# lotus-data/lotus

Hardware: NVIDIA H100
Metric: sem_sim_join queries/sec (1M x 768, K=32) (higher is better)
Workload: dtype bf16

## Files before the change

### lotus_b200/csrc/knn_filter_sm90.cu

```cuda
#include <cuda.h>

#include "common.cuh"

namespace b2 {

namespace {

constexpr int BLOCK_M = 128;
constexpr int BLOCK_N = 256;
constexpr int WG_M = 64;
constexpr int KB_BYTES = 64;
constexpr int KSTEPS = 2;
constexpr int STAGE_A_BYTES = BLOCK_M * KB_BYTES;
constexpr int STAGE_B_BYTES = BLOCK_N * KB_BYTES;
constexpr int STAGE_BYTES = STAGE_A_BYTES + STAGE_B_BYTES;
constexpr int NUM_THREADS = 384;
constexpr int CONSUMER_WARPS = 8;
constexpr int MAX_STAGES = 8;
constexpr int SMEM_LIMIT = 232448;
constexpr int SMEM_ALIGN_SLACK = 1024;
constexpr int BAR_BYTES = 256;
constexpr int FILTER_CL = 4;
constexpr int FILTER_CL_MIN_NTILES = 32;
constexpr int FILTER_MAX_K = 1000;

constexpr int PEND = 16;
constexpr int PEND_FLUSH = 8;
__host__ __device__ constexpr int list_set_stride(int kph) { return kph * BLOCK_M + 16; }
constexpr int PEND_SET_STRIDE = PEND * BLOCK_M + 16;
__host__ __device__ constexpr int list_bytes(int kp) { return 2  * 2  * 4 * (list_set_stride(kp / 2) + PEND_SET_STRIDE); }
constexpr int XP_STRIDE = 17;
constexpr int XP_WARP_FLOATS = 16 * XP_STRIDE;
__host__ __device__ constexpr int misc_bytes() { return CONSUMER_WARPS * XP_WARP_FLOATS * 4 + BAR_BYTES + SMEM_ALIGN_SLACK; }
__host__ __device__ constexpr int num_stages(int kp) {
    const int s = (SMEM_LIMIT - list_bytes(kp) - misc_bytes()) / STAGE_BYTES;
    return s > MAX_STAGES ? MAX_STAGES : s;
}
__host__ __device__ constexpr int smem_bytes(int kp) { return num_stages(kp) * STAGE_BYTES + list_bytes(kp) + misc_bytes(); }

__device__ __forceinline__ uint32_t smem_u32(const void* p) { return (uint32_t)__cvta_generic_to_shared(p); }

__device__ __forceinline__ void mbar_init(uint64_t* bar, uint32_t count) {
    asm volatile("mbarrier.init.shared::cta.b64 [%0], %1;" ::"r"(smem_u32(bar)), "r"(count) : "memory");
}
__device__ __forceinline__ void mbar_arrive_expect_tx(uint64_t* bar, uint32_t bytes) {
    asm volatile("mbarrier.arrive.expect_tx.shared::cta.b64 _, [%0], %1;" ::"r"(smem_u32(bar)), "r"(bytes) : "memory");
}
__device__ __forceinline__ void mbar_arrive(uint64_t* bar) {
    asm volatile("mbarrier.arrive.shared::cta.b64 _, [%0];" ::"r"(smem_u32(bar)) : "memory");
}
__device__ __forceinline__ void mbar_arrive_cluster(uint64_t* bar, uint32_t cta) {
    uint32_t remote;
    asm volatile("mapa.shared::cluster.u32 %0, %1, %2;" : "=r"(remote) : "r"(smem_u32(bar)), "r"(cta));
    asm volatile("mbarrier.arrive.shared::cluster.b64 _, [%0];" ::"r"(remote) : "memory");
}
template <bool SUSPEND>
__device__ __forceinline__ void mbar_wait_impl(uint64_t* bar, uint32_t parity) {
    const uint32_t addr = smem_u32(bar);
    uint32_t done = 0;
    uint32_t spins = 0;
    long long t_start = 0;
    while (true) {
        if constexpr (SUSPEND) {
            asm volatile(
                "{\n\t.reg .pred p;\n\t"
                "mbarrier.try_wait.parity.shared::cta.b64 p, [%1], %2, %3;\n\t"
                "selp.u32 %0, 1, 0, p;\n\t}"
                : "=r"(done)
                : "r"(addr), "r"(parity), "r"(20000u)
                : "memory");
        } else {
            asm volatile(
                "{\n\t.reg .pred p;\n\t"
                "mbarrier.try_wait.parity.shared::cta.b64 p, [%1], %2;\n\t"
                "selp.u32 %0, 1, 0, p;\n\t}"
                : "=r"(done)
                : "r"(addr), "r"(parity)
                : "memory");
        }
        if (done) break;
        if ((++spins & 0x3ffu) == 0) {
            const long long now = clock64();
            if (t_start == 0) t_start = now;
            else if (now - t_start > 8000000000LL) __trap();
        }
    }
}
__device__ __forceinline__ void mbar_wait(uint64_t* bar, uint32_t parity) { mbar_wait_impl<true>(bar, parity); }
__device__ __forceinline__ void mbar_wait_spin(uint64_t* bar, uint32_t parity) { mbar_wait_impl<false>(bar, parity); }
__device__ __forceinline__ void fence_barrier_init() { asm volatile("fence.mbarrier_init.release.cluster;" ::: "memory"); }

__device__ __forceinline__ void tma_load_2d(void* smem_dst, const CUtensorMap* tmap, uint64_t* bar, int c0, int c1) {
    asm volatile(
        "cp.async.bulk.tensor.2d.shared::cluster.global.mbarrier::complete_tx::bytes [%0], [%1, {%3, %4}], [%2];" ::"r"(
            smem_u32(smem_dst)),
        "l"(reinterpret_cast<uint64_t>(tmap)), "r"(smem_u32(bar)), "r"(c0), "r"(c1)
        : "memory");
}
__device__ __forceinline__ void tma_load_2d_multicast(void* smem_dst, const CUtensorMap* tmap, uint64_t* bar, int c0, int c1,
                                                      uint16_t mask) {
    asm volatile(
        "cp.async.bulk.tensor.2d.shared::cluster.global.mbarrier::complete_tx::bytes.multicast::cluster [%0], [%1, {%3, %4}], [%2], %5;" ::"r"(
            smem_u32(smem_dst)),
        "l"(reinterpret_cast<uint64_t>(tmap)), "r"(smem_u32(bar)), "r"(c0), "r"(c1), "h"(mask)
        : "memory");
}
__device__ __forceinline__ void tma_prefetch_desc(const CUtensorMap* tmap) {
    asm volatile("prefetch.tensormap [%0];" ::"l"(reinterpret_cast<uint64_t>(tmap)) : "memory");
}
__device__ __forceinline__ uint32_t cluster_ctarank() {
    uint32_t r;
    asm volatile("mov.u32 %0, %%cluster_ctarank;" : "=r"(r));
    return r;
}
__device__ __forceinline__ void cluster_sync_all() {
    asm volatile("barrier.cluster.arrive.release.aligned;\n\tbarrier.cluster.wait.acquire.aligned;" ::: "memory");
}
template <uint32_t N>
__device__ __forceinline__ void setmaxnreg_inc() { asm volatile("setmaxnreg.inc.sync.aligned.u32 %0;" ::"n"(N)); }
template <uint32_t N>
__device__ __forceinline__ void setmaxnreg_dec() { asm volatile("setmaxnreg.dec.sync.aligned.u32 %0;" ::"n"(N)); }

__device__ __forceinline__ uint64_t make_sw64_desc(uint32_t smem_addr) {
    uint64_t desc = 0;
    desc |= (uint64_t)((smem_addr & 0x3FFFFu) >> 4);
    desc |= (uint64_t)1 << 16;
    desc |= (uint64_t)((8 * KB_BYTES) >> 4) << 32;
    desc |= (uint64_t)2 << 62;
    return desc;
}
__device__ __forceinline__ void wgmma_fence() { asm volatile("wgmma.fence.sync.aligned;" ::: "memory"); }
__device__ __forceinline__ void wgmma_commit() { asm volatile("wgmma.commit_group.sync.aligned;" ::: "memory"); }
template <int N>
__device__ __forceinline__ void wgmma_wait() { asm volatile("wgmma.wait_group.sync.aligned %0;" ::"n"(N) : "memory"); }
__device__ __forceinline__ void acc_fence(float (&d)[128]) {
#pragma unroll
    for (int i = 0; i < 128; ++i) asm volatile("" : "+f"(d[i])::"memory");
}

enum class Op { BF16, F16, TF32 };
__host__ __device__ constexpr int op_bytes(Op op) { return op == Op::TF32 ? 4 : 2; }

#define B2_WGMMA_64X256(SHAPE_TYPES, IMM_TAIL)                                                                               \
    asm volatile("{\n\t.reg .pred p;\n\tsetp.ne.b32 p, %130, 0;\n\t"                                                   \
                 "wgmma.mma_async.sync.aligned." SHAPE_TYPES " "                                                           \
                 "{%0, %1, %2, %3, %4, %5, %6, %7, %8, %9, %10, %11, %12, %13, %14, %15, %16, %17, %18, %19, %20, %21, %22, %23, %24, %25, %26, %27, %28, %29, %30, %31, %32, %33, %34, %35, %36, %37, %38, %39, %40, %41, %42, %43, %44, %45, %46, %47, %48, %49, %50, %51, %52, %53, %54, %55, %56, %57, %58, %59, %60, %61, %62, %63, %64, %65, %66, %67, %68, %69, %70, %71, %72, %73, %74, %75, %76, %77, %78, %79, %80, %81, %82, %83, %84, %85, %86, %87, %88, %89, %90, %91, %92, %93, %94, %95, %96, %97, %98, %99, %100, %101, %102, %103, %104, %105, %106, %107, %108, %109, %110, %111, %112, %113, %114, %115, %116, %117, %118, %119, %120, %121, %122, %123, %124, %125, %126, %127}" ", %128, %129, p, 1, 1" IMM_TAIL ";\n\t}"                                                          \
                 : "+f"(d[0]), "+f"(d[1]), "+f"(d[2]), "+f"(d[3]), "+f"(d[4]), "+f"(d[5]), "+f"(d[6]), "+f"(d[7]), "+f"(d[8]), "+f"(d[9]), "+f"(d[10]), "+f"(d[11]), "+f"(d[12]), "+f"(d[13]), "+f"(d[14]), "+f"(d[15]), "+f"(d[16]), "+f"(d[17]), "+f"(d[18]), "+f"(d[19]), "+f"(d[20]), "+f"(d[21]), "+f"(d[22]), "+f"(d[23]), "+f"(d[24]), "+f"(d[25]), "+f"(d[26]), "+f"(d[27]), "+f"(d[28]), "+f"(d[29]), "+f"(d[30]), "+f"(d[31]), "+f"(d[32]), "+f"(d[33]), "+f"(d[34]), "+f"(d[35]), "+f"(d[36]), "+f"(d[37]), "+f"(d[38]), "+f"(d[39]), "+f"(d[40]), "+f"(d[41]), "+f"(d[42]), "+f"(d[43]), "+f"(d[44]), "+f"(d[45]), "+f"(d[46]), "+f"(d[47]), "+f"(d[48]), "+f"(d[49]), "+f"(d[50]), "+f"(d[51]), "+f"(d[52]), "+f"(d[53]), "+f"(d[54]), "+f"(d[55]), "+f"(d[56]), "+f"(d[57]), "+f"(d[58]), "+f"(d[59]), "+f"(d[60]), "+f"(d[61]), "+f"(d[62]), "+f"(d[63]), "+f"(d[64]), "+f"(d[65]), "+f"(d[66]), "+f"(d[67]), "+f"(d[68]), "+f"(d[69]), "+f"(d[70]), "+f"(d[71]), "+f"(d[72]), "+f"(d[73]), "+f"(d[74]), "+f"(d[75]), "+f"(d[76]), "+f"(d[77]), "+f"(d[78]), "+f"(d[79]), "+f"(d[80]), "+f"(d[81]), "+f"(d[82]), "+f"(d[83]), "+f"(d[84]), "+f"(d[85]), "+f"(d[86]), "+f"(d[87]), "+f"(d[88]), "+f"(d[89]), "+f"(d[90]), "+f"(d[91]), "+f"(d[92]), "+f"(d[93]), "+f"(d[94]), "+f"(d[95]), "+f"(d[96]), "+f"(d[97]), "+f"(d[98]), "+f"(d[99]), "+f"(d[100]), "+f"(d[101]), "+f"(d[102]), "+f"(d[103]), "+f"(d[104]), "+f"(d[105]), "+f"(d[106]), "+f"(d[107]), "+f"(d[108]), "+f"(d[109]), "+f"(d[110]), "+f"(d[111]), "+f"(d[112]), "+f"(d[113]), "+f"(d[114]), "+f"(d[115]), "+f"(d[116]), "+f"(d[117]), "+f"(d[118]), "+f"(d[119]), "+f"(d[120]), "+f"(d[121]), "+f"(d[122]), "+f"(d[123]), "+f"(d[124]), "+f"(d[125]), "+f"(d[126]), "+f"(d[127])                                                                                                         \
                 : "l"(adesc), "l"(bdesc), "r"(scale_d))

template <Op OP>
__device__ __forceinline__ void wgmma_64x256(float (&d)[128], uint64_t adesc, uint64_t bdesc, uint32_t scale_d) {
    if constexpr (OP == Op::TF32) {
        B2_WGMMA_64X256("m64n256k8.f32.tf32.tf32", "");
    } else if constexpr (OP == Op::F16) {
        B2_WGMMA_64X256("m64n256k16.f32.f16.f16", ", 0, 0");
    } else {
        B2_WGMMA_64X256("m64n256k16.f32.bf16.bf16", ", 0, 0");
    }
}
#undef B2_WGMMA_64X256

struct FilterParams {
    const float* xnorm;
    float* cand_score;
    int32_t* cand_id;
    float* cand_thr;
    int32_t nq;
    int32_t n;
    int32_t num_kb;
    int32_t n_mtiles;
    int32_t n_munits;
    int32_t n_splits;
    int32_t top1;
    int32_t tiles_per_split;
    int32_t units_whole;
    int32_t n_ntiles;
    int32_t pair_mode, part, nparts, pair_group, pair_items;
    int32_t pair_align;
    float pair_thr;
    int32_t* pair_i;
    int32_t* pair_j;
    unsigned long long* pair_count;
    unsigned long long pair_cap;
};

struct Ring {
    uint8_t* stage_base;
    uint64_t *full_bar, *empty_bar;
};

struct Sched {
    int worker, n_workers;
    int rank;
    int cta;
};
template <int CL>
__device__ __forceinline__ Sched make_sched() {
    Sched sc;
    if constexpr (CL > 1) {
        sc.worker = blockIdx.x >> 1;
        sc.n_workers = gridDim.x >> 1;
        sc.cta = (int)cluster_ctarank();
        sc.rank = CL == 2 ? sc.cta : (sc.cta & 1);
    } else {
        sc.worker = blockIdx.x;
        sc.n_workers = gridDim.x;
        sc.rank = 0;
        sc.cta = 0;
    }
    return sc;
}
__device__ __forceinline__ int num_items(const FilterParams& p) {
    if (p.pair_mode) return p.pair_items;
    return p.units_whole + (p.n_munits - p.units_whole) * p.n_splits;
}
template <int CL>
__device__ __forceinline__ void item_range(const FilterParams& p, const Sched& sc, int item, int& m_tile, int& split, int& t0,
                                           int& t1) {
    if (p.pair_mode) {
        const int grp = item / p.pair_group;
        const int first = (grp * p.nparts + p.part) * p.pair_group;
        const int unit = first + (item - grp * p.pair_group);
        m_tile = CL > 1 ? 2 * unit + sc.rank : unit;
        split = 0;
        const int lead_tile = (p.pair_align ? first : unit) * (CL > 1 ? 2 : 1);
        t0 = (lead_tile * BLOCK_M) / BLOCK_N;
        t1 = p.n_ntiles;
    } else {
        int unit;
        if (item < p.units_whole) {
            unit = item;
            split = 0;
            t0 = 0;
            t1 = p.n_ntiles;
        } else {
            const int j = item - p.units_whole, rem = p.n_munits - p.units_whole;
            unit = p.units_whole + j % rem;
            split = j / rem;
            t0 = split * p.tiles_per_split;
            t1 = min(t0 + p.tiles_per_split, p.n_ntiles);
        }
        m_tile = CL > 1 ? 2 * unit + sc.rank : unit;
    }
}

template <Op OP, int NSTAGES, int CL>
__device__ __forceinline__ void producer_loop(const CUtensorMap* tmap_q, const CUtensorMap* tmap_x, const FilterParams& p,
                                              const Ring& r, const Sched& sc) {
    constexpr int KB_ELEMS = KB_BYTES / op_bytes(OP);
    const int n_items = num_items(p);
    int stage = 0;
    uint32_t phase = 0;
    for (int item = sc.worker; item < n_items; item += sc.n_workers) {
        int m_tile, split, t0, t1;
        item_range<CL>(p, sc, item, m_tile, split, t0, t1);
        for (int t = t0; t < t1; ++t) {
            for (int kb = 0; kb < p.num_kb; ++kb) {
                mbar_wait(&r.empty_bar[stage], phase ^ 1);
                uint8_t* sa = r.stage_base + stage * STAGE_BYTES;
                uint8_t* sb = sa + STAGE_A_BYTES;
                mbar_arrive_expect_tx(&r.full_bar[stage], STAGE_BYTES);
                tma_load_2d(sa, tmap_q, &r.full_bar[stage], kb * KB_ELEMS, m_tile * BLOCK_M);
                if constexpr (CL > 1)
                    tma_load_2d_multicast(sb + sc.cta * (STAGE_B_BYTES / CL), tmap_x, &r.full_bar[stage], kb * KB_ELEMS,
                                          t * BLOCK_N + sc.cta * (BLOCK_N / CL), (uint16_t)((1u << CL) - 1));
                else
                    tma_load_2d(sb, tmap_x, &r.full_bar[stage], kb * KB_ELEMS, t * BLOCK_N);
                if (++stage == NSTAGES) {
                    stage = 0;
                    phase ^= 1;
                }
            }
        }
    }
}

template <int CL>
__device__ __forceinline__ void release_stage(const Ring& r, int s, int cta) {
    __syncwarp();
    if constexpr (CL <= 2) {
        if ((threadIdx.x & 31) == 0) {
            mbar_arrive(&r.empty_bar[s]);
            if constexpr (CL == 2) mbar_arrive_cluster(&r.empty_bar[s], (uint32_t)(cta ^ 1));
        }
    } else {
        const uint32_t lane = threadIdx.x & 31;
        if (lane < CL) mbar_arrive_cluster(&r.empty_bar[s], lane);
    }
}

template <Op OP, int NSTAGES, int CL>
__device__ __forceinline__ void mma_tile(float (&acc)[128], const Ring& r, int num_kb, int g, int cta, int& stage, uint32_t& phase) {
    const uint32_t a_off = (uint32_t)(g * WG_M * KB_BYTES);
    int prev = -1;
    for (int kb = 0; kb < num_kb; ++kb) {
        mbar_wait_spin(&r.full_bar[stage], phase);
        const uint32_t sa = smem_u32(r.stage_base + stage * STAGE_BYTES);
        const uint64_t adesc = make_sw64_desc(sa + a_off);
        const uint64_t bdesc = make_sw64_desc(sa + STAGE_A_BYTES);
        wgmma_fence();
#pragma unroll
        for (int k = 0; k < KSTEPS; ++k)
            wgmma_64x256<OP>(acc, adesc + (uint64_t)(2 * k), bdesc + (uint64_t)(2 * k), (kb | k) != 0 ? 1u : 0u);
        wgmma_commit();
        if (prev >= 0) {
            wgmma_wait<1>();
            release_stage<CL>(r, prev, cta);
        }
        prev = stage;
        if (++stage == NSTAGES) {
            stage = 0;
            phase ^= 1;
        }
    }
    wgmma_wait<0>();
    acc_fence(acc);
    release_stage<CL>(r, prev, cta);
}

template <int NSTAGES, int CL>
__device__ __forceinline__ Ring setup_ring(uint8_t* smem, const CUtensorMap* tmap_q, const CUtensorMap* tmap_x) {
    Ring r;
    r.stage_base = smem;
    uint64_t* bars = reinterpret_cast<uint64_t*>(smem + NSTAGES * STAGE_BYTES);
    r.full_bar = bars;
    r.empty_bar = bars + NSTAGES;
    if (threadIdx.x == 0) {
        tma_prefetch_desc(tmap_q);
        tma_prefetch_desc(tmap_x);
        for (int s = 0; s < NSTAGES; ++s) {
            mbar_init(&r.full_bar[s], 1);
            mbar_init(&r.empty_bar[s], CL * CONSUMER_WARPS);
        }
        fence_barrier_init();
    }
    if constexpr (CL > 1) cluster_sync_all();
    else __syncthreads();
    return r;
}

template <int CL>
__device__ __forceinline__ void teardown_ring() {
    __syncwarp();
    if constexpr (CL > 1) cluster_sync_all();
}

__device__ __forceinline__ uint8_t* align_smem(uint8_t* raw) {
    const uint32_t a = smem_u32(raw);
    return raw + ((1024u - (a & 1023u)) & 1023u);
}

template <int KP>
__device__ __forceinline__ void list_insert(float* sc, int32_t* id, float s, int32_t idx, float& thr, int& minpos) {
    const bool filling = minpos < 0;
    const int pos = filling ? -minpos - 1 : minpos;
    sc[pos * BLOCK_M] = s;
    id[pos * BLOCK_M] = idx;
    if (filling && pos + 1 < KP) {
        minpos = -(pos + 1) - 1;
        return;
    }
    static_assert(KP % 4 == 0, "list length must be a multiple of 4");
    float m[4];
    int mp[4];
#pragma unroll
    for (int c = 0; c < 4; ++c) {
        m[c] = sc[c * BLOCK_M];
        mp[c] = c;
    }
#pragma unroll
    for (int p = 4; p < KP; p += 4) {
#pragma unroll
        for (int c = 0; c < 4; ++c) {
            const float v = sc[(p + c) * BLOCK_M];
            if (v < m[c]) {
                m[c] = v;
                mp[c] = p + c;
            }
        }
    }
    if (m[1] < m[0] || (m[1] == m[0] && mp[1] < mp[0])) { m[0] = m[1]; mp[0] = mp[1]; }
    if (m[3] < m[2] || (m[3] == m[2] && mp[3] < mp[2])) { m[2] = m[3]; mp[2] = mp[3]; }
    if (m[2] < m[0] || (m[2] == m[0] && mp[2] < mp[0])) { m[0] = m[2]; mp[0] = mp[2]; }
    thr = m[0];
    minpos = mp[0];
}

template <int KP>
__device__ __forceinline__ float2 flush_pending(float* my_sc, int32_t* my_id, const float* pend_sc, const int32_t* pend_id,
                                             int cnt, float thr, int minpos) {
    int mx = cnt;
#pragma unroll
    for (int off = 16; off >= 1; off >>= 1) mx = max(mx, __shfl_xor_sync(0xffffffffu, mx, off));
    for (int i = 0; i < mx; ++i) {
        if (i < cnt) {
            const float s = pend_sc[i * BLOCK_M];
            if (s > thr) list_insert<KP>(my_sc, my_id, s, pend_id[i * BLOCK_M], thr, minpos);
        }
        __syncwarp();
    }
    return make_float2(thr, __int_as_float(minpos));
}

template <bool IS_L2>
__device__ __forceinline__ void prepare8(float (&v)[8], int idx0, int valid, const float* xnorm) {
#pragma unroll
    for (int j = 0; j < 8; ++j) {
        if (j < valid) {
            if constexpr (IS_L2) v[j] = fmaf(2.f, v[j], -__ldg(xnorm + idx0 + j));
        } else {
            v[j] = -INFINITY;
        }
    }
}

template <int KPH>
__device__ __forceinline__ void process8(const float (&v)[8], int idx0, float* my_sc, int32_t* my_id, float* pend_sc,
                                         int32_t* pend_id, float& thr, int& minpos, int& cnt) {
#pragma unroll
    for (int j = 0; j < 8; ++j) {
        if (v[j] > thr) {
            pend_sc[cnt * BLOCK_M] = v[j];
            pend_id[cnt * BLOCK_M] = idx0 + j;
            ++cnt;
        }
    }
    if (__any_sync(0xffffffffu, cnt >= PEND_FLUSH)) {
        const float2 fr = flush_pending<KPH>(my_sc, my_id, pend_sc, pend_id, cnt, thr, minpos);
        thr = fr.x;
        minpos = __float_as_int(fr.y);
        cnt = 0;
    }
}

__device__ __forceinline__ void process8_top2(const float (&v)[8], int idx0, float& b1, float& b2, float& b3, int32_t& i1,
                                              int32_t& i2) {
#pragma unroll
    for (int j = 0; j < 8; ++j) {
        const float s = v[j];
        const int32_t id = idx0 + j;
        const bool c3 = s > b3, c2 = s > b2, c1 = s > b1;
        b3 = c2 ? b2 : (c3 ? s : b3);
        i2 = c1 ? i1 : (c2 ? id : i2);
        b2 = c1 ? b1 : (c2 ? s : b2);
        i1 = c1 ? id : i1;
        b1 = c1 ? s : b1;
    }
}

template <int KP, bool IS_L2, Op OP, int CL, bool TOP1 = false>
__global__ void __launch_bounds__(NUM_THREADS, 1)
knn_filter_kernel(const __grid_constant__ CUtensorMap tmap_q, const __grid_constant__ CUtensorMap tmap_x,
                  const FilterParams p) {
    constexpr int NSTAGES = num_stages(KP);
    static_assert(NSTAGES >= 2, "not enough shared memory for the operand ring");
    constexpr int KPH = KP / 2;
    static_assert(KPH % 4 == 0, "list length must allow float4 write-out");
    constexpr int LSET = list_set_stride(KPH);

    extern __shared__ uint8_t smem_raw[];
    uint8_t* smem = align_smem(smem_raw);
    float* xpose = reinterpret_cast<float*>(smem + NSTAGES * STAGE_BYTES + BAR_BYTES);
    float* list_sc = xpose + CONSUMER_WARPS * XP_WARP_FLOATS;
    int32_t* list_id = reinterpret_cast<int32_t*>(list_sc + 2 * LSET);
    float* pend_sc_base = reinterpret_cast<float*>(list_id + 2 * LSET);
    int32_t* pend_id_base = reinterpret_cast<int32_t*>(pend_sc_base + 2 * PEND_SET_STRIDE);
    const int warp = threadIdx.x >> 5;
    const int lane = threadIdx.x & 31;
    const Ring ring = setup_ring<NSTAGES, CL>(smem, &tmap_q, &tmap_x);
    const int n_items = num_items(p);
    const Sched sc = make_sched<CL>();

    if (warp < 4) {
        setmaxnreg_dec<40>();
        if (threadIdx.x == 0) producer_loop<OP, NSTAGES, CL>(&tmap_q, &tmap_x, p, ring, sc);
    } else {
        setmaxnreg_inc<232>();
        const int g = (warp >> 2) - 1;
        const int wq = warp & 3;
        const int rr = lane & 15, e = lane >> 4;
        const int row = g * WG_M + wq * 16 + rr;
        float* my_sc = list_sc + e * LSET + row;
        int32_t* my_id = list_id + e * LSET + row;
        float* pend_sc = pend_sc_base + e * PEND_SET_STRIDE + row;
        int32_t* pend_id = pend_id_base + e * PEND_SET_STRIDE + row;
        float* xs = xpose + (warp - 4) * XP_WARP_FLOATS;
        const int fr = lane >> 2, fc = 2 * (lane & 3);
        int stage = 0;
        uint32_t phase = 0;
        float acc[128];
        for (int item = sc.worker; item < n_items; item += sc.n_workers) {
            int m_tile, split, t0, t1;
            item_range<CL>(p, sc, item, m_tile, split, t0, t1);
            if constexpr (!TOP1) {
#pragma unroll 4
                for (int i = 0; i < KPH; ++i) {
                    my_sc[i * BLOCK_M] = -INFINITY;
                    my_id[i * BLOCK_M] = -1;
                }
            }
            float thr = -INFINITY;
            int minpos = -1;
            int cnt = 0;
            float b1 = -INFINITY, b2 = -INFINITY, b3 = -INFINITY;
            int32_t i1 = -1, i2 = -1;
            float gthr[2][2] = {{-INFINITY, -INFINITY}, {-INFINITY, -INFINITY}};
            for (int t = t0; t < t1; ++t) {
                mma_tile<OP, NSTAGES, CL>(acc, ring, p.num_kb, g, sc.cta, stage, phase);
                const int col0 = t * BLOCK_N;
                const int ncols = min(BLOCK_N, p.n - col0);
#pragma unroll
                for (int c = 0; c < BLOCK_N / 16; ++c) {
                    if constexpr (!TOP1) {
                        bool hit = false;
#pragma unroll
                        for (int jj = 0; jj < 2; ++jj) {
#pragma unroll
                            for (int h = 0; h < 4; ++h) {
                                const int off = 16 * c + 8 * jj + fc + (h & 1);
                                float s = acc[(2 * c + jj) * 4 + h];
                                if constexpr (IS_L2) {
                                    if (off < ncols) s = fmaf(2.f, s, -__ldg(p.xnorm + col0 + off));
                                }
                                hit |= off < ncols && s > gthr[h >> 1][jj];
                            }
                        }
                        if (!__any_sync(0xffffffffu, hit)) continue;
                    }
                    __syncwarp();
#pragma unroll
                    for (int jj = 0; jj < 2; ++jj) {
                        const int a = (2 * c + jj) * 4;
                        xs[fr * XP_STRIDE + 8 * jj + fc] = acc[a];
                        xs[fr * XP_STRIDE + 8 * jj + fc + 1] = acc[a + 1];
                        xs[(fr + 8) * XP_STRIDE + 8 * jj + fc] = acc[a + 2];
                        xs[(fr + 8) * XP_STRIDE + 8 * jj + fc + 1] = acc[a + 3];
                    }
                    __syncwarp();
                    float v[8];
#pragma unroll
                    for (int j = 0; j < 8; ++j) v[j] = xs[rr * XP_STRIDE + 8 * e + j];
                    const int off = 16 * c + 8 * e;
                    prepare8<IS_L2>(v, col0 + off, ncols - off, p.xnorm);
                    if constexpr (TOP1) {
                        process8_top2(v, col0 + off, b1, b2, b3, i1, i2);
                    } else {
                        process8<KPH>(v, col0 + off, my_sc, my_id, pend_sc, pend_id, thr, minpos, cnt);
#pragma unroll
                        for (int h = 0; h < 2; ++h) {
#pragma unroll
                            for (int s = 0; s < 2; ++s) gthr[h][s] = __shfl_sync(0xffffffffu, thr, fr + 8 * h + 16 * s);
                        }
                    }
                }
            }
            if constexpr (TOP1) {
#pragma unroll 4
                for (int i = 2; i < KPH; ++i) {
                    my_sc[i * BLOCK_M] = -INFINITY;
                    my_id[i * BLOCK_M] = -1;
                }
                my_sc[0 * BLOCK_M] = b1;
                my_id[0 * BLOCK_M] = i1;
                my_sc[1 * BLOCK_M] = b2;
                my_id[1 * BLOCK_M] = i2;
                thr = b3;
            } else {
                const float2 fl = flush_pending<KPH>(my_sc, my_id, pend_sc, pend_id, cnt, thr, minpos);
                thr = fl.x;
                minpos = __float_as_int(fl.y);
                cnt = 0;
            }
            const int q = m_tile * BLOCK_M + row;
            if (q < p.nq) {
                const size_t lidx = ((size_t)q * p.n_splits + split) * 2 + e;
                float4* osc = reinterpret_cast<float4*>(p.cand_score + lidx * KPH);
                int4* oid = reinterpret_cast<int4*>(p.cand_id + lidx * KPH);
#pragma unroll 4
                for (int i = 0; i < KPH / 4; ++i) {
                    osc[i] = make_float4(my_sc[(4 * i + 0) * BLOCK_M], my_sc[(4 * i + 1) * BLOCK_M],
                                         my_sc[(4 * i + 2) * BLOCK_M], my_sc[(4 * i + 3) * BLOCK_M]);
                    oid[i] = make_int4(my_id[(4 * i + 0) * BLOCK_M], my_id[(4 * i + 1) * BLOCK_M],
                                       my_id[(4 * i + 2) * BLOCK_M], my_id[(4 * i + 3) * BLOCK_M]);
                }
                p.cand_thr[lidx] = thr;
            }
        }
    }

    teardown_ring<CL>();
}

constexpr int PAIR_STAGES = MAX_STAGES;
constexpr int PAIR_SMEM = PAIR_STAGES * STAGE_BYTES + BAR_BYTES + SMEM_ALIGN_SLACK;

template <Op OP, int CL>
__global__ void __launch_bounds__(NUM_THREADS, 1)
pair_filter_kernel(const __grid_constant__ CUtensorMap tmap_q, const __grid_constant__ CUtensorMap tmap_x, const FilterParams p) {
    extern __shared__ uint8_t smem_raw[];
    uint8_t* smem = align_smem(smem_raw);
    const int warp = threadIdx.x >> 5;
    const int lane = threadIdx.x & 31;
    const Ring ring = setup_ring<PAIR_STAGES, CL>(smem, &tmap_q, &tmap_x);
    const int n_items = num_items(p);
    const Sched sc = make_sched<CL>();
    if (warp < 4) {
        setmaxnreg_dec<40>();
        if (threadIdx.x == 0) producer_loop<OP, PAIR_STAGES, CL>(&tmap_q, &tmap_x, p, ring, sc);
    } else {
        setmaxnreg_inc<232>();
        const int g = (warp >> 2) - 1;
        const int wq = warp & 3;
        const float thr = p.pair_thr;
        int stage = 0;
        uint32_t phase = 0;
        float acc[128];
        for (int item = sc.worker; item < n_items; item += sc.n_workers) {
            int m_tile, split, t0, t1;
            item_range<CL>(p, sc, item, m_tile, split, t0, t1);
            const int gi0 = m_tile * BLOCK_M + g * WG_M + wq * 16 + (lane >> 2);
            for (int t = t0; t < t1; ++t) {
                mma_tile<OP, PAIR_STAGES, CL>(acc, ring, p.num_kb, g, sc.cta, stage, phase);
                const int col0 = t * BLOCK_N + 2 * (lane & 3);
                float mx = acc[0];
#pragma unroll
                for (int i = 1; i < 128; ++i) mx = fmaxf(mx, acc[i]);
                if (mx > thr && gi0 < p.n) {
#pragma unroll
                    for (int i = 0; i < 128; ++i) {
                        const int gi = gi0 + 8 * ((i >> 1) & 1);
                        const int gj = col0 + 8 * (i >> 2) + (i & 1);
                        if (acc[i] > thr && gj > gi && gj < p.n && gi < p.n) {
                            const unsigned long long pos = atomicAdd(p.pair_count, 1ull);
                            if (pos < p.pair_cap) {
                                p.pair_i[pos] = gi;
                                p.pair_j[pos] = gj;
                            }
                        }
                    }
                }
            }
        }
    }
    teardown_ring<CL>();
}

typedef CUresult (*PFN_encodeTiled)(CUtensorMap*, CUtensorMapDataType, cuuint32_t, void*, const cuuint64_t*,
                                    const cuuint64_t*, const cuuint32_t*, const cuuint32_t*, CUtensorMapInterleave,
                                    CUtensorMapSwizzle, CUtensorMapL2promotion, CUtensorMapFloatOOBfill);

PFN_encodeTiled get_encode_fn() {
    static PFN_encodeTiled fn = nullptr;
    if (fn) return fn;
    void* p = nullptr;
    cudaDriverEntryPointQueryResult qres;
    cudaError_t e = cudaGetDriverEntryPoint("cuTensorMapEncodeTiled", &p, cudaEnableDefault, &qres);
    if (e != cudaSuccess || qres != cudaDriverEntryPointSuccess || !p) {
        set_error("cuTensorMapEncodeTiled is not available from the driver (%s)", cudaGetErrorString(e));
        return nullptr;
    }
    fn = reinterpret_cast<PFN_encodeTiled>(p);
    return fn;
}

Op filter_op(int filt_dtype) {
    switch (filt_dtype) {
        case B2_F32: return Op::TF32;
        case B2_BF16: return Op::BF16;
        default: return Op::F16;
    }
}
CUtensorMapDataType tma_data_type(Op op) {
    switch (op) {
        case Op::TF32: return CU_TENSOR_MAP_DATA_TYPE_FLOAT32;
        case Op::BF16: return CU_TENSOR_MAP_DATA_TYPE_BFLOAT16;
        default: return CU_TENSOR_MAP_DATA_TYPE_FLOAT16;
    }
}

int make_tmap(CUtensorMap* map, const void* base, Op op, int64_t rows, int64_t cols, int64_t pitch, int box_rows) {
    PFN_encodeTiled enc = get_encode_fn();
    if (!enc) return B2_ECUDA;
    const int esz = op_bytes(op);
    cuuint64_t gdim[2] = {(cuuint64_t)cols, (cuuint64_t)rows};
    cuuint64_t gstride[1] = {(cuuint64_t)pitch * esz};
    cuuint32_t box[2] = {(cuuint32_t)(KB_BYTES / esz), (cuuint32_t)box_rows};
    cuuint32_t estr[2] = {1, 1};
    if ((reinterpret_cast<uintptr_t>(base) & 15) != 0 || (gstride[0] & 15) != 0) {
        set_error("TMA operand not 16-byte aligned (base %p, pitch %lld B)", base, (long long)gstride[0]);
        return B2_EINVAL;
    }
    CUresult r = enc(map, tma_data_type(op), 2,
                     const_cast<void*>(base), gdim, gstride, box, estr, CU_TENSOR_MAP_INTERLEAVE_NONE,
                     CU_TENSOR_MAP_SWIZZLE_64B, CU_TENSOR_MAP_L2_PROMOTION_L2_256B, CU_TENSOR_MAP_FLOAT_OOB_FILL_NONE);
    if (r != CUDA_SUCCESS) {
        set_error("cuTensorMapEncodeTiled failed with CUresult %d (rows %lld cols %lld pitch %lld)", (int)r,
                  (long long)rows, (long long)cols, (long long)pitch);
        return B2_ECUDA;
    }
    return B2_OK;
}

template <typename Kern>
int launch_cluster(Kern kern, int grid, int smem, int cl, const CUtensorMap& tq, const CUtensorMap& tx, const FilterParams& p,
                   cudaStream_t stream) {
    B2_CUDA(cudaFuncSetAttribute(kern, cudaFuncAttributeMaxDynamicSharedMemorySize, smem));
    cudaLaunchConfig_t cfg = {};
    cfg.gridDim = dim3((unsigned)grid);
    cfg.blockDim = dim3(NUM_THREADS);
    cfg.dynamicSmemBytes = smem;
    cfg.stream = stream;
    cudaLaunchAttribute attr[1];
    attr[0].id = cudaLaunchAttributeClusterDimension;
    attr[0].val.clusterDim.x = (unsigned)cl;
    attr[0].val.clusterDim.y = 1;
    attr[0].val.clusterDim.z = 1;
    cfg.attrs = attr;
    cfg.numAttrs = 1;
    B2_CUDA(cudaLaunchKernelEx(&cfg, kern, tq, tx, p));
    B2_LAUNCH_CHECK();
    g_stats[ST_FILTER_LAUNCHES]++;
    return B2_OK;
}

template <int KP, bool IS_L2, Op OP, int CL, bool TOP1 = false>
int launch_variant(const CUtensorMap& tq, const CUtensorMap& tx, const FilterParams& p, int grid, cudaStream_t stream) {
    return launch_cluster(knn_filter_kernel<KP, IS_L2, OP, CL, TOP1>, grid, smem_bytes(KP), CL, tq, tx, p, stream);
}

template <int KP, bool IS_L2, int CL, bool TOP1 = false>
int launch_op(Op op, const CUtensorMap& tq, const CUtensorMap& tx, const FilterParams& p, int grid, cudaStream_t stream) {
    switch (op) {
        case Op::TF32: return launch_variant<KP, IS_L2, Op::TF32, CL, TOP1>(tq, tx, p, grid, stream);
        case Op::BF16: return launch_variant<KP, IS_L2, Op::BF16, CL, TOP1>(tq, tx, p, grid, stream);
        default: return launch_variant<KP, IS_L2, Op::F16, CL, TOP1>(tq, tx, p, grid, stream);
    }
}

template <int KP, int CL>
int launch_kp(bool is_l2, Op op, const CUtensorMap& tq, const CUtensorMap& tx, const FilterParams& p, int grid,
              cudaStream_t stream) {
    return is_l2 ? launch_op<KP, true, CL>(op, tq, tx, p, grid, stream) : launch_op<KP, false, CL>(op, tq, tx, p, grid, stream);
}

template <int CL>
int launch_top1(bool is_l2, Op op, const CUtensorMap& tq, const CUtensorMap& tx, const FilterParams& p, int grid,
                cudaStream_t stream) {
    return is_l2 ? launch_op<16, true, CL, true>(op, tq, tx, p, grid, stream)
                 : launch_op<16, false, CL, true>(op, tq, tx, p, grid, stream);
}

template <int CL>
int launch_cl(int kp, bool is_l2, Op op, const CUtensorMap& tq, const CUtensorMap& tx, const FilterParams& p, int grid,
              cudaStream_t stream) {
    switch (kp) {
        case 16: return launch_kp<16, CL>(is_l2, op, tq, tx, p, grid, stream);
        case 32: return launch_kp<32, CL>(is_l2, op, tq, tx, p, grid, stream);
        case 64: return launch_kp<64, CL>(is_l2, op, tq, tx, p, grid, stream);
        case 72: return launch_kp<72, CL>(is_l2, op, tq, tx, p, grid, stream);
        default: set_error("internal: unsupported candidate capacity %d", kp); return B2_EINVAL;
    }
}

template <typename Kern>
int co_resident_clusters(Kern kern, int smem, int cl, int* n) {
    B2_CUDA(cudaFuncSetAttribute(kern, cudaFuncAttributeMaxDynamicSharedMemorySize, smem));
    cudaLaunchConfig_t cfg = {};
    cfg.gridDim = dim3((unsigned)cl);
    cfg.blockDim = dim3(NUM_THREADS);
    cfg.dynamicSmemBytes = smem;
    cudaLaunchAttribute attr[1];
    attr[0].id = cudaLaunchAttributeClusterDimension;
    attr[0].val.clusterDim.x = (unsigned)cl;
    attr[0].val.clusterDim.y = 1;
    attr[0].val.clusterDim.z = 1;
    cfg.attrs = attr;
    cfg.numAttrs = 1;
    *n = 0;
    B2_CUDA(cudaOccupancyMaxActiveClusters(n, kern, &cfg));
    if (*n <= 0) {
        set_error("the filter kernel fits no cluster of %d CTAs (%d B of shared memory each)", cl, smem);
        return B2_ECUDA;
    }
    return B2_OK;
}

template <int KP>
int co_resident_filter_clusters(int cl, int* n) {
    switch (cl) {
        case 1: return co_resident_clusters(knn_filter_kernel<KP, false, Op::BF16, 1>, smem_bytes(KP), cl, n);
        case 2: return co_resident_clusters(knn_filter_kernel<KP, false, Op::BF16, 2>, smem_bytes(KP), cl, n);
        default: return co_resident_clusters(knn_filter_kernel<KP, false, Op::BF16, FILTER_CL>, smem_bytes(KP), cl, n);
    }
}

}

int sm_count(int device) {
    static int cached[64] = {0};
    if (device >= 0 && device < 64 && cached[device]) return cached[device];
    int n = 132;
    cudaDeviceGetAttribute(&n, cudaDevAttrMultiProcessorCount, device);
    if (device >= 0 && device < 64) cached[device] = n;
    return n;
}

int filter_kp_for_k(int k) {
    if (k <= 6) return 16;
    if (k <= 16) return 32;
    if (k <= 40) return 64;
    if (k <= FILTER_MAX_K) return 72;
    return 0;
}

int filter_min_splits_for_k(int k) { return k <= 40 ? 1 : (int)ceil_div(k, 36); }

int filter_cluster(int64_t nq, int64_t n, bool top1) {
    static int mode = -1;
    if (mode < 0) {
        const char* e = getenv("B2_FILTER_2CTA");
        mode = e ? (atoi(e) != 0 ? 1 : 0) : 1;
    }
    const int cl = top1 || ceil_div(n, BLOCK_N) < FILTER_CL_MIN_NTILES ? 2 : FILTER_CL;
    return mode == 1 && ceil_div(nq, BLOCK_M) >= cl ? cl : 1;
}

int filter_workers(int device, int kp, int cl, int* workers) {
    static int cached[64][3][4] = {};
    const int ki = kp == 16 ? 0 : kp == 32 ? 1 : kp == 64 ? 2 : 3;
    const int ci = cl == 1 ? 0 : cl == 2 ? 1 : 2;
    int* slot = (device >= 0 && device < 64) ? &cached[device][ci][ki] : nullptr;
    if (slot && *slot) {
        *workers = *slot;
        return B2_OK;
    }
    switch (kp) {
        case 16: B2_TRY(co_resident_filter_clusters<16>(cl, workers)); break;
        case 32: B2_TRY(co_resident_filter_clusters<32>(cl, workers)); break;
        case 64: B2_TRY(co_resident_filter_clusters<64>(cl, workers)); break;
        case 72: B2_TRY(co_resident_filter_clusters<72>(cl, workers)); break;
        default: set_error("internal: unsupported candidate capacity %d", kp); return B2_EINVAL;
    }
    if (cl > 2) *workers *= cl / 2;
    if (slot) *slot = *workers;
    return B2_OK;
}

int filter_choose_splits(int64_t nq, int64_t n, int workers, int cl, bool top1, int min_splits, int* units_whole) {
    if (units_whole) *units_whole = 0;
    const int64_t n_mtiles = ceil_div(nq, BLOCK_M);
    const int64_t n_units = cl > 1 ? ceil_div(n_mtiles, 2) : n_mtiles;
    auto split_units = [cl](int64_t u) { return cl > 2 ? u + (u & 1) : u; };
    const int64_t n_ntiles = ceil_div(n, BLOCK_N);
    const double kWarmupTiles = top1 ? 1.0 : 13.0;
    double best_cost = 1e300;
    int best = 0;
    for (int s = std::max(1, min_splits); s <= 256 && s <= n_ntiles; ++s) {
        const int64_t tps = ceil_div(n_ntiles, s);
        if (ceil_div(n_ntiles, tps) != s) continue;
        const int64_t items = split_units(n_units) * s;
        const int64_t waves = ceil_div(items, workers);
        const double cost = (double)waves * ((double)tps + kWarmupTiles) * (1.0 + 0.004 * s);
        if (cost < best_cost - 1e-9) {
            best_cost = cost;
            best = s;
        }
    }
    const int64_t waves_a = n_units / workers;
    if (units_whole && min_splits <= 1 && waves_a >= 1) {
        const int64_t ua = waves_a * workers, rem = n_units - ua;
        const double cost_a = (double)waves_a * ((double)n_ntiles + kWarmupTiles);
        double best2 = 1e300;
        int s2 = 1;
        if (rem == 0) {
            best2 = cost_a;
        } else {
            for (int s = 1; s <= 256 && s <= n_ntiles; ++s) {
                const int64_t tps = ceil_div(n_ntiles, s);
                if (ceil_div(n_ntiles, tps) != s) continue;
                const int64_t waves_b = ceil_div(split_units(rem) * s, workers);
                const double cost = (cost_a + (double)waves_b * ((double)tps + kWarmupTiles)) * (1.0 + 0.002 * s);
                if (cost < best2 - 1e-9) {
                    best2 = cost;
                    s2 = s;
                }
            }
        }
        if (best2 < best_cost - 1e-9) {
            *units_whole = (int)ua;
            return s2;
        }
    }
    return best;
}

int launch_knn_filter(const MatView& X, const void* q_filt, int64_t q_pitch, int64_t nq, int metric, int kp,
                      int n_splits, int cluster, int workers, float* cand_score, int32_t* cand_id, float* cand_thr,
                      cudaStream_t stream, bool top1, int units_whole) {
    if (nq <= 0 || X.n <= 0) return B2_OK;
    if (X.n > 0x7fffff00LL || nq > 0x7fffff00LL) {
        set_error("matrix too large for 32-bit row ids (n=%lld nq=%lld)", (long long)X.n, (long long)nq);
        return B2_ERANGE;
    }
    const Op op = filter_op(X.filt_dtype);
    const int kb_elems = KB_BYTES / op_bytes(op);
    CUtensorMap tq, tx;
    const int64_t op_cols = X.d;
    B2_TRY(make_tmap(&tq, q_filt, op, nq, op_cols, q_pitch, BLOCK_M));
    B2_TRY(make_tmap(&tx, X.filt, op, X.n, op_cols, X.filt_pitch, BLOCK_N / cluster));
    FilterParams p;
    p.xnorm = X.norm2;
    p.cand_score = cand_score;
    p.cand_id = cand_id;
    p.cand_thr = cand_thr;
    p.nq = (int32_t)nq;
    p.n = (int32_t)X.n;
    p.num_kb = (int32_t)ceil_div(X.d, kb_elems);
    p.n_mtiles = (int32_t)ceil_div(nq, BLOCK_M);
    p.n_munits = cluster > 1 ? (p.n_mtiles + 1) / 2 : p.n_mtiles;
    p.n_ntiles = (int32_t)ceil_div(X.n, BLOCK_N);
    p.tiles_per_split = (int32_t)ceil_div(p.n_ntiles, n_splits);
    p.n_splits = n_splits;
    p.units_whole = units_whole;
    p.top1 = (top1 && kp == 16) ? 1 : 0;
    p.pair_mode = 0;
// ... 110 lines not shown
```

Measured before the change: 266,400.

## Keep query A-fragments register-resident across N tiles via RS wgmma

```diff
diff --git a/lotus_b200/csrc/knn_filter_sm90.cu b/lotus_b200/csrc/knn_filter_sm90.cu
--- a/lotus_b200/csrc/knn_filter_sm90.cu
+++ b/lotus_b200/csrc/knn_filter_sm90.cu
@@ -11,6 +11,7 @@
 constexpr int WG_M = 64;
 constexpr int KB_BYTES = 64;
 constexpr int KSTEPS = 2;
+constexpr int KB_AREGS = 4 * KSTEPS;
 constexpr int STAGE_A_BYTES = BLOCK_M * KB_BYTES;
 constexpr int STAGE_B_BYTES = BLOCK_N * KB_BYTES;
 constexpr int STAGE_BYTES = STAGE_A_BYTES + STAGE_B_BYTES;
@@ -22,6 +23,7 @@
 constexpr int BAR_BYTES = 256;
 constexpr int FILTER_CL = 4;
 constexpr int FILTER_CL_MIN_NTILES = 32;
+constexpr int FILTER_RES_KB = 6;
 constexpr int FILTER_MAX_K = 1000;
 
 constexpr int PEND = 16;
@@ -141,12 +143,21 @@
 enum class Op { BF16, F16, TF32 };
 __host__ __device__ constexpr int op_bytes(Op op) { return op == Op::TF32 ? 4 : 2; }
 
+#define B2_WGMMA_D                                                                                                           \
+    "{%0, %1, %2, %3, %4, %5, %6, %7, %8, %9, %10, %11, %12, %13, %14, %15, %16, %17, %18, %19, %20, %21, %22, %23, %24, %25, %26, %27, %28, %29, %30, %31, %32, %33, %34, %35, %36, %37, %38, %39, %40, %41, %42, %43, %44, %45, %46, %47, %48, %49, %50, %51, %52, %53, %54, %55, %56, %57, %58, %59, %60, %61, %62, %63, %64, %65, %66, %67, %68, %69, %70, %71, %72, %73, %74, %75, %76, %77, %78, %79, %80, %81, %82, %83, %84, %85, %86, %87, %88, %89, %90, %91, %92, %93, %94, %95, %96, %97, %98, %99, %100, %101, %102, %103, %104, %105, %106, %107, %108, %109, %110, %111, %112, %113, %114, %115, %116, %117, %118, %119, %120, %121, %122, %123, %124, %125, %126, %127}"
+#define B2_WGMMA_D_OPS                                                                                                       \
+    "+f"(d[0]), "+f"(d[1]), "+f"(d[2]), "+f"(d[3]), "+f"(d[4]), "+f"(d[5]), "+f"(d[6]), "+f"(d[7]), "+f"(d[8]), "+f"(d[9]), "+f"(d[10]), "+f"(d[11]), "+f"(d[12]), "+f"(d[13]), "+f"(d[14]), "+f"(d[15]), "+f"(d[16]), "+f"(d[17]), "+f"(d[18]), "+f"(d[19]), "+f"(d[20]), "+f"(d[21]), "+f"(d[22]), "+f"(d[23]), "+f"(d[24]), "+f"(d[25]), "+f"(d[26]), "+f"(d[27]), "+f"(d[28]), "+f"(d[29]), "+f"(d[30]), "+f"(d[31]), "+f"(d[32]), "+f"(d[33]), "+f"(d[34]), "+f"(d[35]), "+f"(d[36]), "+f"(d[37]), "+f"(d[38]), "+f"(d[39]), "+f"(d[40]), "+f"(d[41]), "+f"(d[42]), "+f"(d[43]), "+f"(d[44]), "+f"(d[45]), "+f"(d[46]), "+f"(d[47]), "+f"(d[48]), "+f"(d[49]), "+f"(d[50]), "+f"(d[51]), "+f"(d[52]), "+f"(d[53]), "+f"(d[54]), "+f"(d[55]), "+f"(d[56]), "+f"(d[57]), "+f"(d[58]), "+f"(d[59]), "+f"(d[60]), "+f"(d[61]), "+f"(d[62]), "+f"(d[63]), "+f"(d[64]), "+f"(d[65]), "+f"(d[66]), "+f"(d[67]), "+f"(d[68]), "+f"(d[69]), "+f"(d[70]), "+f"(d[71]), "+f"(d[72]), "+f"(d[73]), "+f"(d[74]), "+f"(d[75]), "+f"(d[76]), "+f"(d[77]), "+f"(d[78]), "+f"(d[79]), "+f"(d[80]), "+f"(d[81]), "+f"(d[82]), "+f"(d[83]), "+f"(d[84]), "+f"(d[85]), "+f"(d[86]), "+f"(d[87]), "+f"(d[88]), "+f"(d[89]), "+f"(d[90]), "+f"(d[91]), "+f"(d[92]), "+f"(d[93]), "+f"(d[94]), "+f"(d[95]), "+f"(d[96]), "+f"(d[97]), "+f"(d[98]), "+f"(d[99]), "+f"(d[100]), "+f"(d[101]), "+f"(d[102]), "+f"(d[103]), "+f"(d[104]), "+f"(d[105]), "+f"(d[106]), "+f"(d[107]), "+f"(d[108]), "+f"(d[109]), "+f"(d[110]), "+f"(d[111]), "+f"(d[112]), "+f"(d[113]), "+f"(d[114]), "+f"(d[115]), "+f"(d[116]), "+f"(d[117]), "+f"(d[118]), "+f"(d[119]), "+f"(d[120]), "+f"(d[121]), "+f"(d[122]), "+f"(d[123]), "+f"(d[124]), "+f"(d[125]), "+f"(d[126]), "+f"(d[127])
 #define B2_WGMMA_64X256(SHAPE_TYPES, IMM_TAIL)                                                                               \
     asm volatile("{\n\t.reg .pred p;\n\tsetp.ne.b32 p, %130, 0;\n\t"                                                   \
-                 "wgmma.mma_async.sync.aligned." SHAPE_TYPES " "                                                           \
-                 "{%0, %1, %2, %3, %4, %5, %6, %7, %8, %9, %10, %11, %12, %13, %14, %15, %16, %17, %18, %19, %20, %21, %22, %23, %24, %25, %26, %27, %28, %29, %30, %31, %32, %33, %34, %35, %36, %37, %38, %39, %40, %41, %42, %43, %44, %45, %46, %47, %48, %49, %50, %51, %52, %53, %54, %55, %56, %57, %58, %59, %60, %61, %62, %63, %64, %65, %66, %67, %68, %69, %70, %71, %72, %73, %74, %75, %76, %77, %78, %79, %80, %81, %82, %83, %84, %85, %86, %87, %88, %89, %90, %91, %92, %93, %94, %95, %96, %97, %98, %99, %100, %101, %102, %103, %104, %105, %106, %107, %108, %109, %110, %111, %112, %113, %114, %115, %116, %117, %118, %119, %120, %121, %122, %123, %124, %125, %126, %127}" ", %128, %129, p, 1, 1" IMM_TAIL ";\n\t}"                                                          \
-                 : "+f"(d[0]), "+f"(d[1]), "+f"(d[2]), "+f"(d[3]), "+f"(d[4]), "+f"(d[5]), "+f"(d[6]), "+f"(d[7]), "+f"(d[8]), "+f"(d[9]), "+f"(d[10]), "+f"(d[11]), "+f"(d[12]), "+f"(d[13]), "+f"(d[14]), "+f"(d[15]), "+f"(d[16]), "+f"(d[17]), "+f"(d[18]), "+f"(d[19]), "+f"(d[20]), "+f"(d[21]), "+f"(d[22]), "+f"(d[23]), "+f"(d[24]), "+f"(d[25]), "+f"(d[26]), "+f"(d[27]), "+f"(d[28]), "+f"(d[29]), "+f"(d[30]), "+f"(d[31]), "+f"(d[32]), "+f"(d[33]), "+f"(d[34]), "+f"(d[35]), "+f"(d[36]), "+f"(d[37]), "+f"(d[38]), "+f"(d[39]), "+f"(d[40]), "+f"(d[41]), "+f"(d[42]), "+f"(d[43]), "+f"(d[44]), "+f"(d[45]), "+f"(d[46]), "+f"(d[47]), "+f"(d[48]), "+f"(d[49]), "+f"(d[50]), "+f"(d[51]), "+f"(d[52]), "+f"(d[53]), "+f"(d[54]), "+f"(d[55]), "+f"(d[56]), "+f"(d[57]), "+f"(d[58]), "+f"(d[59]), "+f"(d[60]), "+f"(d[61]), "+f"(d[62]), "+f"(d[63]), "+f"(d[64]), "+f"(d[65]), "+f"(d[66]), "+f"(d[67]), "+f"(d[68]), "+f"(d[69]), "+f"(d[70]), "+f"(d[71]), "+f"(d[72]), "+f"(d[73]), "+f"(d[74]), "+f"(d[75]), "+f"(d[76]), "+f"(d[77]), "+f"(d[78]), "+f"(d[79]), "+f"(d[80]), "+f"(d[81]), "+f"(d[82]), "+f"(d[83]), "+f"(d[84]), "+f"(d[85]), "+f"(d[86]), "+f"(d[87]), "+f"(d[88]), "+f"(d[89]), "+f"(d[90]), "+f"(d[91]), "+f"(d[92]), "+f"(d[93]), "+f"(d[94]), "+f"(d[95]), "+f"(d[96]), "+f"(d[97]), "+f"(d[98]), "+f"(d[99]), "+f"(d[100]), "+f"(d[101]), "+f"(d[102]), "+f"(d[103]), "+f"(d[104]), "+f"(d[105]), "+f"(d[106]), "+f"(d[107]), "+f"(d[108]), "+f"(d[109]), "+f"(d[110]), "+f"(d[111]), "+f"(d[112]), "+f"(d[113]), "+f"(d[114]), "+f"(d[115]), "+f"(d[116]), "+f"(d[117]), "+f"(d[118]), "+f"(d[119]), "+f"(d[120]), "+f"(d[121]), "+f"(d[122]), "+f"(d[123]), "+f"(d[124]), "+f"(d[125]), "+f"(d[126]), "+f"(d[127])                                                                                                         \
+                 "wgmma.mma_async.sync.aligned." SHAPE_TYPES " " B2_WGMMA_D ", %128, %129, p, 1, 1" IMM_TAIL ";\n\t}"         \
+                 : B2_WGMMA_D_OPS                                                                                          \
                  : "l"(adesc), "l"(bdesc), "r"(scale_d))
+#define B2_WGMMA_64X256_RS(SHAPE_TYPES, IMM_TAIL)                                                                            \
+    asm volatile("{\n\t.reg .pred p;\n\tsetp.ne.b32 p, %133, 0;\n\t"                                                   \
+                 "wgmma.mma_async.sync.aligned." SHAPE_TYPES " " B2_WGMMA_D ", {%128, %129, %130, %131}, %132, p, 1, 1"   \
+                 IMM_TAIL ";\n\t}"                                                                                         \
+                 : B2_WGMMA_D_OPS                                                                                          \
+                 : "r"(a[0]), "r"(a[1]), "r"(a[2]), "r"(a[3]), "l"(bdesc), "r"(scale_d))
 
 template <Op OP>
 __device__ __forceinline__ void wgmma_64x256(float (&d)[128], uint64_t adesc, uint64_t bdesc, uint32_t scale_d) {
@@ -158,7 +169,45 @@
         B2_WGMMA_64X256("m64n256k16.f32.bf16.bf16", ", 0, 0");
     }
 }
+template <Op OP>
+__device__ __forceinline__ void wgmma_64x256_rs(float (&d)[128], const uint32_t* a, uint64_t bdesc, uint32_t scale_d) {
+    if constexpr (OP == Op::TF32) {
+        B2_WGMMA_64X256_RS("m64n256k8.f32.tf32.tf32", "");
+    } else if constexpr (OP == Op::F16) {
+        B2_WGMMA_64X256_RS("m64n256k16.f32.f16.f16", ", 0");
+    } else {
+        B2_WGMMA_64X256_RS("m64n256k16.f32.bf16.bf16", ", 0");
+    }
+}
+#undef B2_WGMMA_64X256_RS
 #undef B2_WGMMA_64X256
+#undef B2_WGMMA_D_OPS
+#undef B2_WGMMA_D
+
+template <Op OP>
+__device__ __forceinline__ void load_a_frag(uint32_t (&a)[KB_AREGS], uint32_t slice) {
+    const int lane = threadIdx.x & 31;
+    const int r0 = ((threadIdx.x >> 5) & 3) * 16;
+    auto chunk_addr = [slice](int r, int c) { return slice + (uint32_t)(r * KB_BYTES + ((c ^ ((r >> 1) & 3)) << 4)); };
+#pragma unroll
+    for (int k = 0; k < KSTEPS; ++k) {
+        uint32_t* f = a + 4 * k;
+        if constexpr (OP == Op::TF32) {
+#pragma unroll
+            for (int j = 0; j < 4; ++j) {
+                const uint32_t addr = chunk_addr(r0 + (lane >> 2) + 8 * (j & 1), 2 * k + (j >> 1)) + 4 * (lane & 3);
+                asm volatile("ld.shared.b32 %0, [%1];" : "=r"(f[j]) : "r"(addr) : "memory");
+            }
+        } else {
+            const int m = lane >> 3;
+            const uint32_t addr = chunk_addr(r0 + 8 * (m & 1) + (lane & 7), 2 * k + (m >> 1));
+            asm volatile("ldmatrix.sync.aligned.m8n8.x4.shared.b16 {%0, %1, %2, %3}, [%4];"
+                         : "=r"(f[0]), "=r"(f[1]), "=r"(f[2]), "=r"(f[3])
+                         : "r"(addr)
+                         : "memory");
+        }
+    }
+}
 
 struct FilterParams {
     const float* xnorm;
@@ -244,7 +293,7 @@
     }
 }
 
-template <Op OP, int NSTAGES, int CL>
+template <Op OP, int NSTAGES, int CL, int RES_KB>
 __device__ __forceinline__ void producer_loop(const CUtensorMap* tmap_q, const CUtensorMap* tmap_x, const FilterParams& p,
                                               const Ring& r, const Sched& sc) {
     constexpr int KB_ELEMS = KB_BYTES / op_bytes(OP);
@@ -259,8 +308,9 @@
                 mbar_wait(&r.empty_bar[stage], phase ^ 1);
                 uint8_t* sa = r.stage_base + stage * STAGE_BYTES;
                 uint8_t* sb = sa + STAGE_A_BYTES;
-                mbar_arrive_expect_tx(&r.full_bar[stage], STAGE_BYTES);
-                tma_load_2d(sa, tmap_q, &r.full_bar[stage], kb * KB_ELEMS, m_tile * BLOCK_M);
+                const bool a_resident = t != t0 && kb < RES_KB;
+                mbar_arrive_expect_tx(&r.full_bar[stage], a_resident ? STAGE_B_BYTES : STAGE_BYTES);
+                if (!a_resident) tma_load_2d(sa, tmap_q, &r.full_bar[stage], kb * KB_ELEMS, m_tile * BLOCK_M);
                 if constexpr (CL > 1)
                     tma_load_2d_multicast(sb + sc.cta * (STAGE_B_BYTES / CL), tmap_x, &r.full_bar[stage], kb * KB_ELEMS,
                                           t * BLOCK_N + sc.cta * (BLOCK_N / CL), (uint16_t)((1u << CL) - 1));
@@ -289,11 +339,38 @@
     }
 }
 
-template <Op OP, int NSTAGES, int CL>
-__device__ __forceinline__ void mma_tile(float (&acc)[128], const Ring& r, int num_kb, int g, int cta, int& stage, uint32_t& phase) {
+template <Op OP, int NSTAGES, int CL, int RES_KB>
+__device__ __forceinline__ void mma_tile(float (&acc)[128], uint32_t (&afrag)[RES_KB > 0 ? RES_KB : 1][KB_AREGS], bool load_a,
+                                         const Ring& r, int num_kb, int g, int cta, int& stage, uint32_t& phase) {
     const uint32_t a_off = (uint32_t)(g * WG_M * KB_BYTES);
     int prev = -1;
-    for (int kb = 0; kb < num_kb; ++kb) {
+    auto retire = [&]() {
+        wgmma_commit();
+        if (prev >= 0) {
+            wgmma_wait<1>();
+            release_stage<CL>(r, prev, cta);
+        }
+        prev = stage;
+        if (++stage == NSTAGES) {
+            stage = 0;
+            phase ^= 1;
+        }
+    };
+#pragma unroll
+    for (int kb = 0; kb < RES_KB; ++kb) {
+        if (kb < num_kb) {
+            mbar_wait_spin(&r.full_bar[stage], phase);
+            const uint32_t sa = smem_u32(r.stage_base + stage * STAGE_BYTES);
+            if (load_a) load_a_frag<OP>(afrag[kb], sa + a_off);
+            const uint64_t bdesc = make_sw64_desc(sa + STAGE_A_BYTES);
+            wgmma_fence();
+#pragma unroll
+            for (int k = 0; k < KSTEPS; ++k)
+                wgmma_64x256_rs<OP>(acc, afrag[kb] + 4 * k, bdesc + (uint64_t)(2 * k), (kb | k) != 0 ? 1u : 0u);
+            retire();
+        }
+    }
+    for (int kb = RES_KB; kb < num_kb; ++kb) {
         mbar_wait_spin(&r.full_bar[stage], phase);
         const uint32_t sa = smem_u32(r.stage_base + stage * STAGE_BYTES);
         const uint64_t adesc = make_sw64_desc(sa + a_off);
@@ -302,16 +379,7 @@
 #pragma unroll
         for (int k = 0; k < KSTEPS; ++k)
             wgmma_64x256<OP>(acc, adesc + (uint64_t)(2 * k), bdesc + (uint64_t)(2 * k), (kb | k) != 0 ? 1u : 0u);
-        wgmma_commit();
-        if (prev >= 0) {
-            wgmma_wait<1>();
-            release_stage<CL>(r, prev, cta);
-        }
-        prev = stage;
-        if (++stage == NSTAGES) {
-            stage = 0;
-            phase ^= 1;
-        }
+        retire();
     }
     wgmma_wait<0>();
     acc_fence(acc);
@@ -457,6 +525,7 @@
     constexpr int KPH = KP / 2;
     static_assert(KPH % 4 == 0, "list length must allow float4 write-out");
     constexpr int LSET = list_set_stride(KPH);
+    constexpr int RES_KB = FILTER_RES_KB;
 
     extern __shared__ uint8_t smem_raw[];
     uint8_t* smem = align_smem(smem_raw);
@@ -473,7 +542,7 @@
 
     if (warp < 4) {
         setmaxnreg_dec<40>();
-        if (threadIdx.x == 0) producer_loop<OP, NSTAGES, CL>(&tmap_q, &tmap_x, p, ring, sc);
+        if (threadIdx.x == 0) producer_loop<OP, NSTAGES, CL, RES_KB>(&tmap_q, &tmap_x, p, ring, sc);
     } else {
         setmaxnreg_inc<232>();
         const int g = (warp >> 2) - 1;
@@ -489,6 +558,7 @@
         int stage = 0;
         uint32_t phase = 0;
         float acc[128];
+        uint32_t afrag[RES_KB][KB_AREGS];
         for (int item = sc.worker; item < n_items; item += sc.n_workers) {
             int m_tile, split, t0, t1;
             item_range<CL>(p, sc, item, m_tile, split, t0, t1);
@@ -506,7 +576,7 @@
             int32_t i1 = -1, i2 = -1;
             float gthr[2][2] = {{-INFINITY, -INFINITY}, {-INFINITY, -INFINITY}};
             for (int t = t0; t < t1; ++t) {
-                mma_tile<OP, NSTAGES, CL>(acc, ring, p.num_kb, g, sc.cta, stage, phase);
+                mma_tile<OP, NSTAGES, CL, RES_KB>(acc, afrag, t == t0, ring, p.num_kb, g, sc.cta, stage, phase);
                 const int col0 = t * BLOCK_N;
                 const int ncols = min(BLOCK_N, p.n - col0);
 #pragma unroll
@@ -606,7 +676,7 @@
     const Sched sc = make_sched<CL>();
     if (warp < 4) {
         setmaxnreg_dec<40>();
-        if (threadIdx.x == 0) producer_loop<OP, PAIR_STAGES, CL>(&tmap_q, &tmap_x, p, ring, sc);
+        if (threadIdx.x == 0) producer_loop<OP, PAIR_STAGES, CL, 0>(&tmap_q, &tmap_x, p, ring, sc);
     } else {
         setmaxnreg_inc<232>();
         const int g = (warp >> 2) - 1;
@@ -615,12 +685,13 @@
         int stage = 0;
         uint32_t phase = 0;
         float acc[128];
+        uint32_t no_afrag[1][KB_AREGS];
         for (int item = sc.worker; item < n_items; item += sc.n_workers) {
             int m_tile, split, t0, t1;
             item_range<CL>(p, sc, item, m_tile, split, t0, t1);
             const int gi0 = m_tile * BLOCK_M + g * WG_M + wq * 16 + (lane >> 2);
             for (int t = t0; t < t1; ++t) {
-                mma_tile<OP, PAIR_STAGES, CL>(acc, ring, p.num_kb, g, sc.cta, stage, phase);
+                mma_tile<OP, PAIR_STAGES, CL, 0>(acc, no_afrag, false, ring, p.num_kb, g, sc.cta, stage, phase);
                 const int col0 = t * BLOCK_N + 2 * (lane & 3);
                 float mx = acc[0];
 #pragma unroll
```

New measurement: 274,800 (median of 6 runs). 1.03x the previous value.
